# AER-RC/RRTMG_LW

Measured on AMD Instinct MI355X. Metric: columns/sec, 72-layer profiles, higher is better.
Workload: dtype f64 (transmittance / tfn codes and their LDS table f32); 1 GPU; 1000000 synthetic 72-layer columns, config 'cloudy' (icld=2: rtrnmr max-random overlap, idrv=0), sharded 1x1000000; ncol_total=1000000, nlay=72, columns_per_gpu=1000000, parallelism=columns/1, gather=none, kdata=stand-in (real k-data absent from the reference mount), sweeps=production

## Files before the change

rrtmg_lw_amd/csrc/kernels.hip:

```cpp
#include <hip/hip_runtime.h>
#include "kissjump.hpp"

#ifdef RRLW_TUNE
#define RRLW_BF_TUNE 1u
#else
#define RRLW_BF_TUNE 0u
#endif
#ifdef RRLW_G256
#define RRLW_BF_G256 8u
#else
#define RRLW_BF_G256 0u
#endif
#if defined(RRLW_LAYER_BLOCK) || defined(RRLW_STAGE_DOUBLES) || defined(RRLW_LAYER_WAVES) || defined(RRLW_LOAD_CHUNK) || defined(RRLW_MINOR_WIN) || \
    defined(RRLW_COLSORT_WIN) || defined(RRLW_SWEEPC_P0) || defined(RRLW_SWEEPC_P2D) || defined(RRLW_SWEEPC_WAVES_CAP) || defined(RRLW_SWEEPC_CODES) || \
    defined(RRLW_SWEEPZ_WAVES_G1) || defined(RRLW_SWEEPZ_WAVES_IDRV) || defined(RRLW_LAYER_STAMPS) || \
    defined(RRLW_DBG_DUMP)
#define RRLW_BF_GEOMETRY 16u
#else
#define RRLW_BF_GEOMETRY 0u
#endif

#include <algorithm>
#include <type_traits>
#include <utility>
// ... 566 lines not shown
};
struct Region {
    Key key; int a, b, rat;
    bool self_, for_;
    int planck_slot;
    bool frac_from_a;
    int nm; Minor m[3];
    int ncfc; int cfc_wx[2];
    Corr corr;
    int mult;
};
constexpr Minor NOM = {A_COL, 0, false, 0, 0, 0, 0, 0};
constexpr Region ZERO_REGION = {K_ZERO, 0, 0, 0, false, false, -1, false, 0, {NOM, NOM, NOM}, 0, {0, 0}, C_NONE, 0};

template <int B> struct BT;
#ifdef RRLW_G256
#define BAND_NG(NG_) 16
#else
#define BAND_NG(NG_) NG_
#endif
#define BAND_TRAITS(B_, NG_, LO, UP) \
    template <> struct BT<B_> { static constexpr int ng = BAND_NG(NG_); static constexpr Region lo = LO; static constexpr Region up = UP; };

#define R1(...) Region{__VA_ARGS__}
BAND_TRAITS(1, 10,
    R1(K_SINGLE, H2O, 0, 0, true, true, -1, false, 1, {{A_BRD_N2, BRD, false, 0, 0, 0, 0, 0}, NOM, NOM}, 0, {0, 0}, C_B1LO, 0),
    R1(K_SINGLE, H2O, 0, 0, false, true, -1, false, 1, {{A_BRD_N2, BRD, false, 0, 0, 0, 0, 0}, NOM, NOM}, 0, {0, 0}, C_B1UP, 0))
BAND_TRAITS(2, 12,
    R1(K_SINGLE, H2O, 0, 0, true, true, -1, false, 0, {NOM, NOM, NOM}, 0, {0, 0}, C_B2LO, 0),
    R1(K_SINGLE, H2O, 0, 0, false, true, -1, false, 0, {NOM, NOM, NOM}, 0, {0, 0}, C_NONE, 0))
BAND_TRAITS(3, 16,
    R1(K_BINARY, H2O, CO2, R_H2OCO2, true, true, 0, false, 1, {{A_ADJ, N2O, true, 2, 1.5, 0.5, 0.65, 0}, NOM, NOM}, 0, {0, 0}, C_NONE, 0),
    R1(K_BINARY, H2O, CO2, R_H2OCO2, false, true, 1, false, 1, {{A_ADJ, N2O, true, 3, 1.5, 0.5, 0.65, 0}, NOM, NOM}, 0, {0, 0}, C_NONE, 0))
BAND_TRAITS(4, 14,
    R1(K_BINARY, H2O, CO2, R_H2OCO2, true, true, 0, false, 0, {NOM, NOM, NOM}, 0, {0, 0}, C_NONE, 0),
    R1(K_BINARY, O3, CO2, R_O3CO2, false, false, 1, false, 0, {NOM, NOM, NOM}, 0, {0, 0}, C_NONE, 4))
BAND_TRAITS(5, 16,
    R1(K_BINARY, H2O, CO2, R_H2OCO2, true, true, 0, false, 1, {{A_COL, O3, true, 2, 0, 0, 0, 0}, NOM, NOM}, 1, {1, 0}, C_NONE, 0),
    R1(K_BINARY, O3, CO2, R_O3CO2, false, false, 1, false, 0, {NOM, NOM, NOM}, 1, {1, 0}, C_NONE, 0))
BAND_TRAITS(6, 8,
    R1(K_SINGLE, H2O, 0, 0, true, true, -1, false, 1, {{A_ADJ, CO2, false, 0, 3.0, 2.0, 0.77, 0}, NOM, NOM}, 2, {2, 3}, C_NONE, 0),
    R1(K_NONE, 0, 0, 0, false, false, -1, true, 0, {NOM, NOM, NOM}, 2, {2, 3}, C_NONE, 0))
BAND_TRAITS(7, 12,
    R1(K_BINARY, H2O, O3, R_H2OO3, true, true, 0, false, 1, {{A_ADJ, CO2, true, 2, 3.0, 3.0, 0.79, 0}, NOM, NOM}, 0, {0, 0}, C_NONE, 0),
    R1(K_SINGLE, O3, 0, 0, false, false, -1, false, 1, {{A_ADJ, CO2, false, 0, 3.0, 2.0, 0.79, 0}, NOM, NOM}, 0, {0, 0}, C_NONE, 7))
BAND_TRAITS(8, 8,
    R1(K_SINGLE, H2O, 0, 0, true, true, -1, false, 3,
       {{A_ADJ, CO2, false, 0, 3.0, 2.0, 0.65, 0}, {A_COL, O3, false, 0, 0, 0, 0, 0}, {A_COL, N2O, false, 0, 0, 0, 0, 0}}, 2, {3, 4}, C_NONE, 0),
    R1(K_SINGLE, O3, 0, 0, false, false, -1, false, 2,
       {{A_ADJ, CO2, false, 0, 3.0, 2.0, 0.65, 0}, {A_COL, N2O, false, 0, 0, 0, 0, 0}, NOM}, 2, {3, 4}, C_NONE, 0))
BAND_TRAITS(9, 12,
    R1(K_BINARY, H2O, CH4, R_H2OCH4, true, true, 0, false, 1, {{A_ADJ, N2O, true, 2, 1.5, 0.5, 0.65, 0}, NOM, NOM}, 0, {0, 0}, C_NONE, 0),
    R1(K_SINGLE, CH4, 0, 0, false, false, -1, false, 1, {{A_ADJ, N2O, false, 0, 1.5, 0.5, 0.65, 0}, NOM, NOM}, 0, {0, 0}, C_NONE, 0))
BAND_TRAITS(10, 6,
    R1(K_SINGLE, H2O, 0, 0, true, true, -1, false, 0, {NOM, NOM, NOM}, 0, {0, 0}, C_NONE, 0),
    R1(K_SINGLE, H2O, 0, 0, false, true, -1, false, 0, {NOM, NOM, NOM}, 0, {0, 0}, C_NONE, 0))
BAND_TRAITS(11, 8,
    R1(K_SINGLE, H2O, 0, 0, true, true, -1, false, 1, {{A_O2, O2, false, 0, 0, 0, 0, 0}, NOM, NOM}, 0, {0, 0}, C_NONE, 0),
    R1(K_SINGLE, H2O, 0, 0, false, true, -1, false, 1, {{A_O2, O2, false, 0, 0, 0, 0, 0}, NOM, NOM}, 0, {0, 0}, C_NONE, 0))
BAND_TRAITS(12, 8,
    R1(K_BINARY, H2O, CO2, R_H2OCO2, true, true, 0, false, 0, {NOM, NOM, NOM}, 0, {0, 0}, C_NONE, 0),
    ZERO_REGION)
BAND_TRAITS(13, 4,
    R1(K_BINARY, H2O, N2O, R_H2ON2O, true, true, 0, false, 2,
       {{A_ADJ, CO2, true, 2, 3.0, 2.0, 0.68, 3.55e-4}, {A_COL, CO, true, 4, 0, 0, 0, 0}, NOM}, 0, {0, 0}, C_NONE, 0),
    R1(K_NONE, 0, 0, 0, false, false, -1, false, 1, {{A_COL, O3, false, 0, 0, 0, 0, 0}, NOM, NOM}, 0, {0, 0}, C_NONE, 0))
BAND_TRAITS(14, 2,
    R1(K_SINGLE, CO2, 0, 0, true, true, -1, false, 0, {NOM, NOM, NOM}, 0, {0, 0}, C_NONE, 0),
    R1(K_SINGLE, CO2, 0, 0, false, false, -1, false, 0, {NOM, NOM, NOM}, 0, {0, 0}, C_NONE, 0))
BAND_TRAITS(15, 2,
    R1(K_BINARY, N2O, CO2, R_N2OCO2, true, true, 0, false, 1, {{A_BRD, BRD, true, 2, 0, 0, 0, 0}, NOM, NOM}, 0, {0, 0}, C_NONE, 0),
    ZERO_REGION)
BAND_TRAITS(16, 2,
    R1(K_BINARY, H2O, CH4, R_H2OCH4, true, true, 0, false, 0, {NOM, NOM, NOM}, 0, {0, 0}, C_NONE, 0),
    R1(K_SINGLE, CH4, 0, 0, false, false, -1, false, 0, {NOM, NOM, NOM}, 0, {0, 0}, C_NONE, 0))
#undef R1

__device__ const double kMult4[16] = {1, 1, 1, 1, 1, 1, 1, 0.92, 0.88, 1.07, 1.1, 0.99, 0.88, 0.943, 1, 1};
__device__ const double kMult7[16] = {1, 1, 1, 1, 1, 0.92, 0.88, 1.07, 1.1, 0.99, 0.855, 1, 1, 1, 1, 1};

struct LayerCoef {
    double f[NFIELD];
    int jp, jt, jt1, indself, indfor, indminor;
};

struct Spec { double speccomb, specparm, fs; int js; };
__device__ __forceinline__ Spec spec_calc(double cola, double rat, double colb, double mult, double oneminus)
{
    Spec s;
    s.speccomb = cola + rat * colb;
    s.specparm = fdiv(cola, s.speccomb);
    if (s.specparm >= oneminus) s.specparm = oneminus;
    const double specmult = mult * s.specparm;
    s.js = 1 + (int)specmult;
    s.fs = specmult - (double)(int)specmult;
    return s;
}

__device__ __forceinline__ void stencil6(double specparm, double fs, double fa, double fb, int &off, double (&w)[6])
{
    if (specparm < 0.125) {
        const double p = fs - 1, p2 = p * p, p4 = p2 * p2;
        const double fk0 = p4, fk1 = 1 - p - 2.0 * p4, fk2 = p + p4;
        off = 0;
        w[0] = fk0 * fa; w[1] = fk1 * fa; w[2] = fk2 * fa; w[3] = fk0 * fb; w[4] = fk1 * fb; w[5] = fk2 * fb;
    } else if (specparm > 0.875) {
        const double p = -fs, p2 = p * p, p4 = p2 * p2;
        const double fk0 = p4, fk1 = 1 - p - 2.0 * p4, fk2 = p + p4;
        off = -1;
        w[0] = fk2 * fa; w[1] = fk1 * fa; w[2] = fk0 * fa; w[3] = fk2 * fb; w[4] = fk1 * fb; w[5] = fk0 * fb;
    } else {
        off = 0;
        w[0] = (1. - fs) * fa; w[1] = fs * fa; w[2] = 0.0; w[3] = (1. - fs) * fb; w[4] = fs * fb; w[5] = 0.0;
    }
}

__host__ __device__ constexpr int region_nrows(const Region &R, bool lower)
{
    int n = 0;
    if (R.key == K_SINGLE) n += 4;
    else if (R.key == K_BINARY) n += lower ? 12 : 8;
    if (R.self_) n += 2;
    if (R.for_) n += 2;
    for (int i = 0; i < R.nm; i++) n += R.m[i].two_d ? 4 : 2;
    n += R.ncfc;
    return n;
}

__host__ __device__ constexpr int region_major_rows(const Region &R, bool lower)
{
    return R.key == K_SINGLE ? 4 : (R.key == K_BINARY ? (lower ? 12 : 8) : 0);
}
__host__ __device__ constexpr int region_minor_base(const Region &R, bool lower, int im)
{
    int n = region_major_rows(R, lower) + (R.self_ ? 2 : 0) + (R.for_ ? 2 : 0);
    for (int i = 0; i < im; i++) n += R.m[i].two_d ? 4 : 2;
    return n;
}

#ifdef RRLW_G256
__host__ __device__ constexpr int band_ng(int B) { return B >= 1 ? 16 : 16; }
#else
__host__ __device__ constexpr int band_ng(int B) { return B == 1 ? 10 : B == 2 ? 12 : B == 3 ? 16 : B == 4 ? 14 : B == 5 ? 16 : B == 6 ? 8 : B == 7 ? 12 :
                                                    B == 8 ? 8 : B == 9 ? 12 : B == 10 ? 6 : B == 11 ? 8 : B == 12 ? 8 : B == 13 ? 4 : 2; }
#endif
__host__ __device__ constexpr int band_nquad(int B) { return (band_ng(B) + 3) / 4; }
__host__ __device__ constexpr int band_qstart(int B)
{
    int s = 0;
    for (int b = 1; b < B; b++) s += band_nquad(b);
    return s;
}
constexpr int NQUAD = band_qstart(17);
__host__ __device__ constexpr int band_g0(int B)
{
    int s = 0;
    for (int b = 1; b < B; b++) s += band_ng(b);
    return s;
}
static_assert(band_g0(17) == NGPT, "g-point table");
static_assert(NQUAD == (NGPT == 140 ? 38 : 64), "quad table");

constexpr int NRATCHI = 6 * 59 + 7 * 59;
__shared__ double s_ratchi[NRATCHI];

template <int N>
struct Rows {
    unsigned off[N > 0 ? N : 1];
    double w[N > 0 ? N : 1];
    unsigned fw;
};

template <int B> constexpr unsigned lo_binary_mask() { return (BT<B>::lo.key == K_BINARY ? 1u << (B - 1) : 0u) | lo_binary_mask<B - 1>(); }
template <> constexpr unsigned lo_binary_mask<0>() { return 0u; }
template <int B> constexpr unsigned up_binary_mask() { return (BT<B>::up.key == K_BINARY ? 1u << (B - 1) : 0u) | up_binary_mask<B - 1>(); }
template <> constexpr unsigned up_binary_mask<0>() { return 0u; }
template <int B> constexpr unsigned up_zero_mask() { return (BT<B>::up.key == K_ZERO ? 1u << (B - 1) : 0u) | up_zero_mask<B - 1>(); }
template <> constexpr unsigned up_zero_mask<0>() { return 0u; }
template <int B> constexpr unsigned up_from_a_mask() { return (BT<B>::up.frac_from_a ? 1u << (B - 1) : 0u) | up_from_a_mask<B - 1>(); }
template <> constexpr unsigned up_from_a_mask<0>() { return 0u; }
constexpr unsigned LO_BINARY = lo_binary_mask<16>(), UP_BINARY = up_binary_mask<16>(), UP_ZERO = up_zero_mask<16>(), UP_FROM_A = up_from_a_mask<16>();
static_assert((UP_BINARY & ~LO_BINARY) == 0u, "fw slots are assigned by the lower region");
__host__ __device__ constexpr int popcnt_c(unsigned v) { int n = 0; for (; v; v &= v - 1) n++; return n; }
constexpr int NFW = popcnt_c(LO_BINARY);
__host__ __device__ constexpr int fw_slot(int B) { return popcnt_c(LO_BINARY & ((1u << (B - 1)) - 1u)); }

template <int B, bool LOWER, int N, int IM>
__device__ __forceinline__ void rows_prep_minor(const DevTables &T, const LayerCoef &C, Rows<N> &rw)
{
    constexpr Region R = LOWER ? BT<B>::lo : BT<B>::up;
    constexpr unsigned ng = BT<B>::ng;
    constexpr Minor M = R.m[IM];
    constexpr int I0 = region_minor_base(R, LOWER, IM);
    const BandLayout &L = T.band[B - 1];
    const double mf = C.f[F_MINORFRAC];
    double amount;
    if constexpr (M.amt == A_COL) amount = C.f[F_COLH2O + M.sp];
    else if constexpr (M.amt == A_BRD_N2) amount = C.f[F_COLBRD] * C.f[F_SCALEMINORN2];
    else if constexpr (M.amt == A_O2) amount = C.f[F_COLO2] * C.f[F_SCALEMINOR];
    else if constexpr (M.amt == A_BRD) amount = C.f[F_COLBRD] * C.f[F_SCALEMINOR];
    else {
        const double colx = C.f[F_COLH2O + M.sp], coldry = C.f[F_COLDRY];
        const double chiref = M.chiconst > 0. ? M.chiconst : s_ratchi[(T.sl.chi - T.sl.rat) + M.sp * 59 + C.jp];
        const double chi = fdiv(colx, coldry);
        const double ratx = fdiv(1.e20 * chi, chiref);
        amount = colx;
        if (ratx > M.thr) amount = (M.base + pow(ratx - M.base, M.expo)) * chiref * coldry * 1.e-20;
    }
    const unsigned slot = (unsigned)(LOWER ? L.minor_lo[IM] : L.minor_up[IM]);
    if constexpr (M.two_d) {
        constexpr unsigned nj = LOWER ? 9 : 5;
        const Spec sm = spec_calc(C.f[F_COLH2O + R.a], T.refrat[B - 1][M.refslot], C.f[F_COLH2O + R.b], LOWER ? 8. : 4., T.oneminus);
        const unsigned r = slot + ((unsigned)(C.indminor - 1) * nj + (unsigned)(sm.js - 1)) * ng;
        rw.off[I0] = r;                    rw.w[I0] = amount * ((1. - mf) * (1. - sm.fs));
        rw.off[I0 + 1] = r + ng;           rw.w[I0 + 1] = amount * ((1. - mf) * sm.fs);
        rw.off[I0 + 2] = r + nj * ng;      rw.w[I0 + 2] = amount * (mf * (1. - sm.fs));
        rw.off[I0 + 3] = r + nj * ng + ng; rw.w[I0 + 3] = amount * (mf * sm.fs);
    } else {
        const unsigned r = slot + (unsigned)(C.indminor - 1) * ng;
        rw.off[I0] = r;          rw.w[I0] = amount * (1. - mf);
        rw.off[I0 + 1] = r + ng; rw.w[I0 + 1] = amount * mf;
    }
}

template <int B, bool LOWER, int N>
__device__ __forceinline__ void rows_prep(const DevTables &T, const LayerCoef &C, Rows<N> &rw)
{
    constexpr Region R = LOWER ? BT<B>::lo : BT<B>::up;
    constexpr unsigned ng = BT<B>::ng;
    const BandLayout &L = T.band[B - 1];
    const int jp = C.jp, jt = C.jt, jt1 = C.jt1;
    const double *rat_tab = s_ratchi;
    rw.fw = 0u;
    if constexpr (R.key == K_ZERO) return;

    double corradj = 1.;
    if constexpr (R.corr == C_B1LO) { if (C.f[F_PAVEL] < 250.) corradj = 1. - 0.15 * (250. - C.f[F_PAVEL]) / 154.4; }
    else if constexpr (R.corr == C_B1UP) corradj = 1. - 0.15 * (C.f[F_PAVEL] / 95.6);
    else if constexpr (R.corr == C_B2LO) corradj = 1. - .05 * (C.f[F_PAVEL] - 100.) / 900.;

    if constexpr (R.key == K_SINGLE) {
        const unsigned r0 = LOWER ? ((jp - 1) * 5 + (jt - 1)) : ((jp - 13) * 5 + (jt - 1));
        const unsigned r1 = LOWER ? (jp * 5 + (jt1 - 1)) : ((jp - 12) * 5 + (jt1 - 1));
        const unsigned tab = (unsigned)(LOWER ? L.absa : L.absb);
        const double colk = C.f[F_COLH2O + R.a];
        rw.off[0] = tab + r0 * ng;       rw.w[0] = colk * C.f[F_FAC00];
        rw.off[1] = tab + (r0 + 1) * ng; rw.w[1] = colk * C.f[F_FAC10];
        rw.off[2] = tab + r1 * ng;       rw.w[2] = colk * C.f[F_FAC01];
        rw.off[3] = tab + (r1 + 1) * ng; rw.w[3] = colk * C.f[F_FAC11];
    } else if constexpr (R.key == K_BINARY) {
        const double cola = C.f[F_COLH2O + R.a], colb = C.f[F_COLH2O + R.b];
        const double rat = rat_tab[R.rat * 59 + (jp - 1)], rat_1 = rat_tab[R.rat * 59 + jp];
        constexpr double mult = LOWER ? 8. : 4.;
        const Spec s = spec_calc(cola, rat, colb, mult, T.oneminus);
        const Spec s1 = spec_calc(cola, rat_1, colb, mult, T.oneminus);
        if constexpr (LOWER) {
            const unsigned tab = (unsigned)L.absa;
            const int ind0 = ((jp - 1) * 5 + (jt - 1)) * 9 + s.js - 1;
            const int ind1 = (jp * 5 + (jt1 - 1)) * 9 + s1.js - 1;
            int so;
            double w6[6];
            stencil6(s.specparm, s.fs, C.f[F_FAC00], C.f[F_FAC10], so, w6);
            unsigned r = tab + (unsigned)(ind0 + so) * ng;
            rw.off[0] = r;           rw.w[0] = s.speccomb * w6[0];
            rw.off[1] = r + ng;      rw.w[1] = s.speccomb * w6[1];
            rw.off[2] = r + 2 * ng;  rw.w[2] = s.speccomb * w6[2];
            rw.off[3] = r + 9 * ng;  rw.w[3] = s.speccomb * w6[3];
            rw.off[4] = r + 10 * ng; rw.w[4] = s.speccomb * w6[4];
            rw.off[5] = r + 11 * ng; rw.w[5] = s.speccomb * w6[5];
            stencil6(s1.specparm, s1.fs, C.f[F_FAC01], C.f[F_FAC11], so, w6);
            r = tab + (unsigned)(ind1 + so) * ng;
            rw.off[6] = r;            rw.w[6] = s1.speccomb * w6[0];
            rw.off[7] = r + ng;       rw.w[7] = s1.speccomb * w6[1];
            rw.off[8] = r + 2 * ng;   rw.w[8] = s1.speccomb * w6[2];
            rw.off[9] = r + 9 * ng;   rw.w[9] = s1.speccomb * w6[3];
            rw.off[10] = r + 10 * ng; rw.w[10] = s1.speccomb * w6[4];
            rw.off[11] = r + 11 * ng; rw.w[11] = s1.speccomb * w6[5];
        } else {
            const unsigned tab = (unsigned)L.absb;
            const unsigned ind0 = ((jp - 13) * 5 + (jt - 1)) * 5 + s.js - 1;
            const unsigned ind1 = ((jp - 12) * 5 + (jt1 - 1)) * 5 + s1.js - 1;
            unsigned r = tab + ind0 * ng;
            rw.off[0] = r;          rw.w[0] = s.speccomb * ((1. - s.fs) * C.f[F_FAC00]);
            rw.off[1] = r + ng;     rw.w[1] = s.speccomb * (s.fs * C.f[F_FAC00]);
            rw.off[2] = r + 5 * ng; rw.w[2] = s.speccomb * ((1. - s.fs) * C.f[F_FAC10]);
            rw.off[3] = r + 6 * ng; rw.w[3] = s.speccomb * (s.fs * C.f[F_FAC10]);
            r = tab + ind1 * ng;
            rw.off[4] = r;          rw.w[4] = s1.speccomb * ((1. - s1.fs) * C.f[F_FAC01]);
            rw.off[5] = r + ng;     rw.w[5] = s1.speccomb * (s1.fs * C.f[F_FAC01]);
            rw.off[6] = r + 5 * ng; rw.w[6] = s1.speccomb * ((1. - s1.fs) * C.f[F_FAC11]);
            rw.off[7] = r + 6 * ng; rw.w[7] = s1.speccomb * (s1.fs * C.f[F_FAC11]);
        }
        const Spec sp = spec_calc(cola, T.refrat[B - 1][R.planck_slot], colb, mult, T.oneminus);
        unsigned q = (unsigned)(sp.fs * 268435456.0 + 0.5);
        if (q > 268435455u) q = 268435455u;
        rw.fw = ((unsigned)sp.js << 28) | q;
    }
    constexpr int IS = region_major_rows(R, LOWER);
    if constexpr (R.self_) {
        const unsigned r = (unsigned)L.selfref + (unsigned)(C.indself - 1) * ng;
        rw.off[IS] = r;          rw.w[IS] = C.f[F_SELFFAC] * (1. - C.f[F_SELFFRAC]);
        rw.off[IS + 1] = r + ng; rw.w[IS + 1] = C.f[F_SELFFAC] * C.f[F_SELFFRAC];
    }
    constexpr int IF = IS + (R.self_ ? 2 : 0);
    if constexpr (R.for_) {
        const unsigned r = (unsigned)L.forref + (unsigned)(C.indfor - 1) * ng;
// ... 1600 lines not shown
__device__ __forceinline__ void sweep_stage_lut(const DevTables &T, unsigned char *smem, int tid, int nth)
{
    const double2 *src = reinterpret_cast<const double2 *>(T.stat + T.sl.lutf);
    double2 *dst = reinterpret_cast<double2 *>(smem);
    constexpr int NLUT = SWEEP_LUT_BYTES / 16;
    for (int i0 = tid; i0 < NLUT; i0 += 8 * nth) {
        double2 v[8];
#pragma unroll
        for (int k = 0; k < 8; k++) v[k] = src[min(i0 + k * nth, NLUT - 1)];
#pragma unroll
        for (int k = 0; k < 8; k++) if (i0 + k * nth < NLUT) dst[i0 + k * nth] = v[k];
    }
}
__device__ __forceinline__ void sweep_stage_band(const DevTables &T, double (*s_pl)[184], double (*s_fr)[16], int B, bool alt16, bool lo_bin, bool up_bin,
                                                 int tid, int nth)
{
    const double *tp = alt16 ? T.stat + T.sl.totplk16 : T.stat + T.sl.totplnk + 181 * (B - 1);
    const double *tq = T.stat + T.sl.totplnk + 181 * 15;
    for (int i = tid; i < 181; i += nth) { s_pl[0][i] = tp[i]; s_pl[1][i] = tq[i]; }
    const int ng = T.band[B - 1].ng, fa = T.band[B - 1].fracrefa, fb = T.band[B - 1].fracrefb;
    const int na = lo_bin ? 9 : 1, nb = up_bin ? 5 : 1;
    for (int i = tid; i < 16 * 16; i += nth) {
        const int r = i >> 4, g = i & 15;
        double v = 0.0;
        if (g < ng) {
            if (r < 9) { if (r < na) v = T.ktab[fa + r * ng + g]; }
            else if (r < 14 && fb >= 0 && r - 9 < nb) v = T.ktab[fb + (r - 9) * ng + g];
        }
        s_fr[r][g] = v;
    }
}
#ifndef RRLW_SWEEPC_P0
#define RRLW_SWEEPC_P0 6, 4, 3, 2
#endif
#ifndef RRLW_SWEEPC_P2D
#define RRLW_SWEEPC_P2D 3, 2, 1, 1
#endif
#ifndef RRLW_SWEEPC_WAVES_CAP
#define RRLW_SWEEPC_WAVES_CAP 4
#endif
__host__ __device__ constexpr int sweepc_waves(int NQ, int PHASE, bool IDRV)
{
    const int row = PHASE == 1 ? 0 : (PHASE == 0 && !IDRV) ? 1 : (PHASE == 2 && IDRV) ? 3 : 2;
    const int tab[4][4] = {{7, 5, 4, 3}, {RRLW_SWEEPC_P0}, {5, 3, 2, 1}, {RRLW_SWEEPC_P2D}};
    const int w = tab[row][NQ - 1];
    return w < RRLW_SWEEPC_WAVES_CAP ? w : RRLW_SWEEPC_WAVES_CAP;
}
constexpr int NGROUP_MAX = 8;
constexpr int SWEEPC_BAND_BYTES = SWEEP_PL_BYTES + SWEEP_FR_BYTES;
__host__ __device__ constexpr int sweepc_nval(int PHASE, bool IDRV) { return (PHASE == 2 ? 2 : 1) * ((IDRV && PHASE != 1) ? 2 : 1); }
#ifndef RRLW_SWEEPC_CODES
#define RRLW_SWEEPC_CODES 2
#endif
constexpr int SWEEPC_LDS_MAX = 160 * 1024;
__host__ __device__ constexpr int sweepc_lds_bytes(int PHASE, bool IDRV, int nb, int nsb, int NT = 1)
{
    return SWEEP_LUT_BYTES + nb * SWEEPC_BAND_BYTES + 2 * sweepc_nval(PHASE, IDRV) * nb * NT * RRLW_SWEEPC_CODES * nsb * 64 * 8;
}
__host__ __device__ constexpr int sweepc_nt(int NQ, int PHASE)
{
    return (NQ == 4 && (PHASE == 2 || PHASE == 0)) ? 2 : 1;
}
__host__ __device__ constexpr int sweepc_group_cap(int NQ)
{
    int cap = 5;
    for (int ph = 0; ph < 3; ph++)
        for (int i = 0; i < 2; i++) {
            if (ph == 1 && i == 1) continue;
            const bool idrv = i == 1;
            const int nt = sweepc_nt(NQ, ph), w = 4 * sweepc_waves(NQ / nt, ph, idrv) / nt;
            if (w < cap) cap = w;
            while (cap > 1 && sweepc_lds_bytes(ph, idrv, cap, 1, nt) > SWEEPC_LDS_MAX) cap--;
        }
    return cap;
}
__host__ __device__ constexpr int sweepc_nsb(int NQ, int PHASE, bool IDRV, int nb)
{
    const int nt = sweepc_nt(NQ, PHASE);
    int nsb = nsb_fit(4 * sweepc_waves(NQ / nt, PHASE, IDRV) / (nb * nt));
    while (nsb > 1 && sweepc_lds_bytes(PHASE, IDRV, nb, nsb, nt) > SWEEPC_LDS_MAX) nsb = nsb_fit(nsb - 1);
    return nsb;
}

template <int G> struct SweepcLev { double tl, tz; unsigned w; };

__device__ __forceinline__ double one_minus(double x)
{
    double t = 1.0 - x;
    asm("" : "+v"(t));
    return t;
}
__device__ __forceinline__ double times(double x, double y)
{
    double t = x * y;
    asm("" : "+v"(t));
    return t;
}

template <int NQ, int PHASE, bool IDRV, int NT = 1, bool SPEC = false>
__global__ __launch_bounds__(256 * sweepc_waves(NQ / NT, PHASE, IDRV), sweepc_waves(NQ / NT, PHASE, IDRV)) void k_sweepc(DevTables T, Workspace W, SweepArgs a)
{
    static_assert(NQ % NT == 0 && (NT == 1 || NT == 2), "threads per band");
    constexpr int G = NQ / NT, NG = 4 * G, NC = RRLW_SWEEPC_CODES;
    constexpr bool DOWN = PHASE != 2, UP = PHASE != 1, TWO = PHASE == 2;
    constexpr int NVAL = sweepc_nval(PHASE, IDRV);
    extern __shared__ __align__(16) unsigned char smem[];
    const int hgrp = (PHASE == 0 && !a.cfree) ? 0 : __builtin_amdgcn_readfirstlane(W.hgrp[(blockIdx.x * blockDim.z) / SORT_GROUP]);
    if (a.cfree && (PHASE == 0) != (hgrp == 0)) return;
    const int tx = threadIdx.x, ty = __builtin_amdgcn_readfirstlane(threadIdx.y), sub = __builtin_amdgcn_readfirstlane(threadIdx.z);
    const int bi = ty / NT, part = ty % NT;
    const int ny = blockDim.y, nb = ny / NT, nsb = blockDim.z, ncw = 64 * nsb;
    const float2 *s_lut = reinterpret_cast<const float2 *>(smem);
    double (*s_pl)[184] = reinterpret_cast<double (*)[184]>(smem + SWEEP_LUT_BYTES + bi * SWEEPC_BAND_BYTES);
    double (*s_fr)[16] = reinterpret_cast<double (*)[16]>(smem + SWEEP_LUT_BYTES + bi * SWEEPC_BAND_BYTES + SWEEP_PL_BYTES);
    double *red = reinterpret_cast<double *>(smem + SWEEP_LUT_BYTES + nb * SWEEPC_BAND_BYTES);
    const int slot = blockIdx.x * nsb + sub;
    const int cblock = (PHASE == 0 && !a.cfree) ? slot : __builtin_amdgcn_readfirstlane(W.order[slot]);
    const int col = cblock * 64 + tx;
    const int bsel = a.split ? (int)blockIdx.y : 0;
    const unsigned long long bands = a.bands >> (4 * bsel);
    const int B = (int)((bands >> (4 * bi)) & 15ull) + 1;
    const bool incol = col < a.ncol;
    const int colc = incol ? col : a.ncol - 1;
    const int quad = __builtin_amdgcn_readfirstlane(band_qstart(B) + part * G);
    const int g0 = NG * part;
    const int pc = pcol(W, colc);
    const size_t gc = (size_t)a.col0 + pc;
    const int nlay = W.nlay, nct = a.nct;
    const size_t ncb = W.ncolb;
    const bool alt16 = (B == 16 && a.istart == 16);
    const bool lo_bin = (LO_BINARY >> (B - 1)) & 1u, up_bin = (UP_BINARY >> (B - 1)) & 1u;
    const bool any_bin = lo_bin || up_bin;
    const int base_up = ((UP_ZERO >> (B - 1)) & 1u) ? 14 : (((UP_FROM_A >> (B - 1)) & 1u) ? 0 : 9);
    sweep_stage_lut(T, smem, (sub * ny + ty) * 64 + tx, 64 * ny * nsb);
    sweep_stage_band(T, s_pl, s_fr, B, alt16, lo_bin, up_bin, (sub * NT + part) * 64 + tx, NT * ncw);
    __syncthreads();
    const int lo = PHASE == 0 ? 1 : hgrp + 1;
    const size_t qstride = (size_t)nlay * ncb;
    const unsigned *__restrict__ sC = W.scr[S_CODE] + (size_t)quad * qstride * CODE_WORDS;
    const unsigned *__restrict__ sFw = W.fw + (size_t)fw_slot(B) * nlay * ncb;
    const bool moved = pmoved(W, colc);
    const double *__restrict__ tlay = moved ? W.tlayc : a.tlay + a.col0;
    const double *__restrict__ tlev = moved ? W.tlevc : a.tlev + a.col0;
    const size_t tstride = moved ? ncb : (size_t)nct;
    const unsigned offc = (unsigned)colc * (unsigned)CODE_BYTES, off8p = (unsigned)colc * 8u, off4 = (unsigned)colc * 4u;
    const size_t pcb = (size_t)W.pcb;
    const size_t gslab = (size_t)(a.group + bsel) * (nlay + 1) * pcb;
    double *__restrict__ gdn1 = W.gdn1 + gslab;
    double *__restrict__ gup1 = W.gup1 + gslab;
    Part2 *__restrict__ gup = W.gup + gslab;
    Part2 *__restrict__ gdp = W.gdp + gslab;
    const unsigned so8 = (unsigned)col * 8u, so16 = (unsigned)col * 16u;
    const int laytrop = W.laytrop[colc];
    const double *tp0 = s_pl[0], *tp1 = s_pl[1];
    double2 *hand = reinterpret_cast<double2 *>(W.hand) + ((size_t)quad * ncb + colc) * 2;
    const size_t hstream = (size_t)NQUAD * ncb * 2;

    constexpr bool SOFF = PHASE != 1;
    const unsigned ncb32 = (unsigned)ncb, tstr32 = (unsigned)tstride;
    auto fill_t = [&](auto bin_tag, int lev, int zoff, SweepcLev<G> &q) {
        const int l = min(max(lev, 1), nlay);
        if constexpr (SOFF) {
            const unsigned r = (unsigned)(l - 1);
            q.tl = bload_f64(row_ptr(tlay, r, tstr32), off8p);
            q.tz = bload_f64(row_ptr(tlev, r + (unsigned)zoff, tstr32), off8p);
            if constexpr (decltype(bin_tag)::value) q.w = bload_u32(sFw, off4, r * ncb32 * 4u);
        } else {
            q.tl = bload_f64(tlay + tstride * (l - 1), off8p);
            q.tz = bload_f64(tlev + tstride * (l - 1 + zoff), off8p);
            if constexpr (decltype(bin_tag)::value) q.w = bload_u32(sFw + (size_t)(l - 1) * ncb, off4);
        }
    };
    auto ld_c = [&](int lev, int k) -> pk4 {
        const int l = min(max(lev, 1), nlay);
        if constexpr (SOFF) return bload_pk4_nt(sC + (size_t)k * qstride * CODE_WORDS, offc, (unsigned)(l - 1) * ncb32 * (unsigned)CODE_BYTES);
        else return bload_pk4_nt(sC + ((size_t)k * qstride + (size_t)(l - 1) * ncb) * CODE_WORDS, offc);
    };
    auto frac_row = [&](int lev, unsigned fwv, double &fpl) -> const double * {
        const bool lower = lev <= laytrop;
        if (any_bin) {
            const unsigned w = (lower ? lo_bin : up_bin) ? fwv : 0x10000000u;
            const int r0 = clampi((lower ? 0 : base_up) + (int)(w >> 28) - 1, 0, 14);
            fpl = (double)(w & 0x0fffffffu) * (1.0 / 268435456.0);
            return &s_fr[r0][g0];
        }
        fpl = 0.0;
        return &s_fr[lower ? 0 : base_up][g0];
    };

    const unsigned rlane = (unsigned)(sub * 64 + tx);
    const unsigned vstride = (unsigned)(ny * NC * ncw), rband = (unsigned)(ty * NC * ncw);
    unsigned bufoff = 0u;
    auto red_put = [&](int c, int val, double v) { red[bufoff + val * vstride + rband + (unsigned)(c * ncw) + rlane] = v; };
    auto round_end = [&](auto dn_tag, int lev0, int nvalid) {
#pragma clang fp contract(off)
        constexpr bool DN = decltype(dn_tag)::value;
        constexpr int NV = DN ? 1 : NVAL;
        __syncthreads();
        for (int c = ty; c < nvalid; c += ny) {
            const int lvl = DN ? lev0 - c - 1 : lev0 + c;
            double sv[NV];
#pragma unroll
            for (int val = 0; val < NV; val++) {
                const double *r = red + (bufoff + val * vstride + (unsigned)(c * ncw) + rlane);
                const bool deriv = IDRV && !DN && val >= (TWO ? 2 : 1);
                double sum = 0.0;
                for (int q = 0; q < nb; q++) {
                    double pq = r[(unsigned)(q * NT * NC * ncw)];
                    if constexpr (NT == 2) pq = pq + r[(unsigned)((q * NT + 1) * NC * ncw)];
                    const int bq = (int)((bands >> (4 * q)) & 15ull);
                    double v = (pq * 0.5) * T.delwave[bq];
                    if (deriv) v = v * T.fluxfac;
                    sum = q == 0 ? v : sum + v;
                    if constexpr (SPEC) {
                        if (incol && !deriv) {
                            const size_t o = spec_at(gc, lvl, bq + 1, nlay, nct);
                            const double f = v * T.fluxfac;
                            if (DN) { a.dflxs[o] = f; if (a.dflxcs) a.dflxcs[o] = f; }
                            else if (val == 0) { a.uflxs[o] = f; if (!TWO && a.uflxcs) a.uflxcs[o] = f; }
                            else if (a.uflxcs) a.uflxcs[o] = f;
                        }
                    }
                }
                sv[val] = sum;
            }
            if (incol) {
                if constexpr (DN) bstore_f64(gdn1 + (size_t)lvl * pcb, so8, sv[0]);
                else {
                    if constexpr (TWO) bstore_f64x2(gup + (size_t)lvl * pcb, so16, sv[0], sv[1]);
                    else bstore_f64(gup1 + (size_t)lvl * pcb, so8, sv[0]);
                    if constexpr (IDRV) bstore_f64x2(gdp + (size_t)lvl * pcb, so16, TWO ? sv[2] : sv[1], TWO ? sv[3] : sv[1]);
                }
            }
        }
        bufoff = bufoff ? 0u : NVAL * vstride;
    };

    double rad[NG], radc[TWO ? NG : 1], drad[IDRV ? NG : 1], dradc[(IDRV && TWO) ? NG : 1];
#pragma unroll
    for (int j = 0; j < NG; j++) rad[j] = 0.0;

    SweepcLev<G> cur;
    cur.w = 0u;
    pk4 cc[G][NC];
    auto level = [&](auto bin_tag, auto dn_tag, int lev, int slot) {
        constexpr bool BIN = decltype(bin_tag)::value, DN = decltype(dn_tag)::value;
        constexpr int dir = DN ? -1 : 1;
        double fpl;
        const double *row = frac_row(lev, cur.w, fpl);
        const double blay = planck_at(tp0, tp0, cur.tl);
        const double dpl = planck_at(tp0, (DN && alt16 && lev == 1) ? tp1 : tp0, cur.tz) - blay;
        fill_t(bin_tag, lev + dir, DN ? 0 : 1, cur);
        double qs[G], qsc[G], qd[G], qdc[G];
#pragma unroll
        for (int k = 0; k < G; k++) {
            pk4 pk;
#pragma unroll
            for (int c = 0; c < NC; c++) if (c == slot) pk = cc[k][c];
            const scr4 ck = unpack4(pk);
            unsigned orw = pk.w[0];
#pragma unroll
            for (int i = 1; i < CODE_WORDS; i++) orw |= pk.w[i];
            const bool thin = wave_all_thin(orw);
            float fa[4], ft[4];
            if (thin) {
#pragma unroll
                for (int jj = 0; jj < 4; jj++) decode_thin(ck.v[jj], fa[jj], ft[jj]);
            } else {
                float2 e[4];
#pragma unroll
                for (int jj = 0; jj < 4; jj++) e[jj] = s_lut[code_index(ck.v[jj])];
#pragma unroll
                for (int jj = 0; jj < 4; jj++) decode_f32(ck.v[jj], e[jj], fa[jj], ft[jj]);
            }
            const pk4 nx = ld_c(lev + NC * dir, k);
#pragma unroll
            for (int c = 0; c < NC; c++) if (c == slot) cc[k][c] = nx;
#pragma unroll
            for (int jj = 0; jj < 4; jj++) {
                const int j = 4 * k + jj;
                const double atr = (double)fa[jj], tfn = (double)ft[jj];
                double fr = row[j];
                if constexpr (BIN) fr = fma(fpl, row[16 + j] - fr, fr);
                const double bb = fr * fma(tfn, dpl, blay);
                rad[j] = fma(bb - rad[j], atr, rad[j]);
                if constexpr (TWO && !DN) radc[j] = fma(bb - radc[j], atr, radc[j]);
                if constexpr (IDRV && !DN) {
                    const double tr = one_minus(atr);
                    drad[j] = times(drad[j], tr);
                    if constexpr (TWO) dradc[j] = times(dradc[j], tr);
                }
            }
            qs[k] = (rad[4 * k] + rad[4 * k + 1]) + (rad[4 * k + 2] + rad[4 * k + 3]);
            if constexpr (TWO && !DN) qsc[k] = (radc[4 * k] + radc[4 * k + 1]) + (radc[4 * k + 2] + radc[4 * k + 3]);
            if constexpr (IDRV && !DN) {
                qd[k] = (drad[4 * k] + drad[4 * k + 1]) + (drad[4 * k + 2] + drad[4 * k + 3]);
                if constexpr (TWO) qdc[k] = (dradc[4 * k] + dradc[4 * k + 1]) + (dradc[4 * k + 2] + dradc[4 * k + 3]);
            }
#pragma unroll
            for (int jj = 0; jj < 4; jj++) {
                asm volatile("" : "+v"(rad[4 * k + jj]));
                if constexpr (TWO && !DN) asm volatile("" : "+v"(radc[4 * k + jj]));
                if constexpr (IDRV && !DN) asm volatile("" : "+v"(drad[4 * k + jj]));
                if constexpr (IDRV && TWO && !DN) asm volatile("" : "+v"(dradc[4 * k + jj]));
            }
        }
        auto tree = [&](const double (&q)[G]) -> double {
            if constexpr (G == 1) return q[0];
            else if constexpr (G == 2) return q[0] + q[1];
            else if constexpr (G == 3) return (q[0] + q[1]) + q[2];
            else return (q[0] + q[1]) + (q[2] + q[3]);
        };
        red_put(slot, 0, tree(qs));
        if constexpr (TWO && !DN) red_put(slot, 1, tree(qsc));
        if constexpr (IDRV && !DN) {
            red_put(slot, TWO ? 2 : 1, tree(qd));
            if constexpr (TWO) red_put(slot, 3, tree(qdc));
        }
    };
    auto sweep = [&](auto bin_tag, auto dn_tag) {
        constexpr bool DN = decltype(dn_tag)::value;
        constexpr int dir = DN ? -1 : 1;
        const int first = DN ? nlay : lo, count = nlay - lo + 1;
#pragma unroll
        for (int c = 0; c < NC; c++) {
            if (c == NC - 1) fill_t(bin_tag, first, DN ? 0 : 1, cur);
#pragma unroll
            for (int k = 0; k < G; k++) cc[k][c] = ld_c(first + c * dir, k);
        }
        int n = 0;
        for (; n + NC <= count; n += NC) {
#pragma unroll
            for (int c = 0; c < NC; c++) level(bin_tag, dn_tag, first + (n + c) * dir, c);
            round_end(dn_tag, first + n * dir, NC);
        }
        const int rem = count - n;
#pragma unroll
        for (int c = 0; c < NC - 1; c++) {
            if (c < rem) level(bin_tag, dn_tag, first + (n + c) * dir, c);
        }
        if (rem > 0) round_end(dn_tag, first + n * dir, rem);
    };
    using std::true_type;
    using std::false_type;

    if constexpr (DOWN) {
        if (incol && ty == 0) bstore_f64(gdn1 + (size_t)nlay * pcb, so8, 0.0);
        if constexpr (SPEC) {
            if (incol && part == 0) {
                const size_t o = spec_at(gc, nlay, B, nlay, nct);
                a.dflxs[o] = 0.0;
                if (a.dflxcs) a.dflxcs[o] = 0.0;
            }
        }
        if (any_bin) sweep(true_type{}, true_type{}); else sweep(false_type{}, true_type{});
    }
    if constexpr (PHASE == 1) {
        if (incol) {
#pragma unroll
            for (int k = 0; k < G; k++) {
                hand[(size_t)k * ncb * 2] = make_double2(rad[4 * k], rad[4 * k + 1]);
                hand[(size_t)k * ncb * 2 + 1] = make_double2(rad[4 * k + 2], rad[4 * k + 3]);
            }
        }
        return;
    }

    if constexpr (PHASE == 0) {
        const double reflect = 1. - a.emis[gc + (size_t)nct * (B - 1)];
        const double pb = W.percol[(size_t)(PC_PLANKBND + B - 1) * ncb + colc];
        const double dpb = IDRV ? W.percol[(size_t)(PC_DPLANKBND + B - 1) * ncb + colc] : 0.0;
        double fpl;
        const double *row = frac_row(1, any_bin ? bload_u32(sFw, off4) : 0u, fpl);
        double usum = 0.0, dusum = 0.0;
#pragma unroll
        for (int j = 0; j < NG; j++) {
            const double fr = any_bin ? fma(fpl, row[16 + j] - row[j], row[j]) : row[j];
            rad[j] = fma(reflect, rad[j], fr * pb);
            usum = usum + rad[j];
            if constexpr (IDRV) { drad[j] = times(fr, dpb); dusum = dusum + drad[j]; }
        }
        if (a.cfree) {
            double qs[G], qd[G];
#pragma unroll
            for (int k = 0; k < G; k++) {
                qs[k] = 0.0; qd[k] = 0.0;
#pragma unroll
                for (int jj = 0; jj < 4; jj++) {
                    qs[k] = qs[k] + rad[4 * k + jj];
                    if constexpr (IDRV) qd[k] = qd[k] + drad[4 * k + jj];
                }
            }
            if constexpr (G == 1) { usum = qs[0]; dusum = qd[0]; }
            else if constexpr (G == 2) { usum = qs[0] + qs[1]; dusum = qd[0] + qd[1]; }
            else if constexpr (G == 3) { usum = (qs[0] + qs[1]) + qs[2]; dusum = (qd[0] + qd[1]) + qd[2]; }
            else { usum = (qs[0] + qs[1]) + (qs[2] + qs[3]); dusum = (qd[0] + qd[1]) + (qd[2] + qd[3]); }
        }
        red_put(0, 0, usum);
        if constexpr (IDRV) red_put(0, 1, dusum);
        round_end(false_type{}, 0, 1);
    } else {
#pragma unroll
        for (int k = 0; k < G; k++) {
            const double2 *h = hand + (size_t)k * ncb * 2;
            const double2 a0 = h[hstream], a1 = h[hstream + 1], c0 = h[2 * hstream], c1 = h[2 * hstream + 1];
            rad[4 * k] = a0.x; rad[4 * k + 1] = a0.y; rad[4 * k + 2] = a1.x; rad[4 * k + 3] = a1.y;
            if constexpr (TWO) { radc[4 * k] = c0.x; radc[4 * k + 1] = c0.y; radc[4 * k + 2] = c1.x; radc[4 * k + 3] = c1.y; }
            if constexpr (IDRV) {
                const double2 d0 = h[3 * hstream], d1 = h[3 * hstream + 1], e0 = h[4 * hstream], e1 = h[4 * hstream + 1];
                drad[4 * k] = d0.x; drad[4 * k + 1] = d0.y; drad[4 * k + 2] = d1.x; drad[4 * k + 3] = d1.y;
                if constexpr (TWO) { dradc[4 * k] = e0.x; dradc[4 * k + 1] = e0.y; dradc[4 * k + 2] = e1.x; dradc[4 * k + 3] = e1.y; }
            }
        }
    }
    if constexpr (UP) {
        if (any_bin) sweep(true_type{}, false_type{}); else sweep(false_type{}, false_type{});
    }
}

__host__ __device__ constexpr int sweepz_nt(int NQ) { return NQ; }
#ifndef RRLW_SWEEPZ_WAVES_G1
#define RRLW_SWEEPZ_WAVES_G1 3
#endif
#ifndef RRLW_SWEEPZ_WAVES_IDRV
#define RRLW_SWEEPZ_WAVES_IDRV 2
#endif
__host__ __device__ constexpr int sweepz_waves(int , bool IDRV = false)
{
    return IDRV ? RRLW_SWEEPZ_WAVES_IDRV : RRLW_SWEEPZ_WAVES_G1;
}
__host__ __device__ constexpr int sweepz_lds_bytes(int nb, int nsb, int NT, bool IDRV = false)
{
    return SWEEP_LUT_BYTES + nb * SWEEPC_BAND_BYTES + 2 * (IDRV ? 4 : 2) * nb * NT * RRLW_SWEEPC_CODES * nsb * 64 * 8;
}
__host__ __device__ constexpr int sweepz_nsb(int NQ, int nb, bool IDRV = false)
{
    const int nt = sweepz_nt(NQ);
    int nsb = nsb_fit(4 * sweepz_waves(NQ, IDRV) / (nb * nt));
    while (nsb > 1 && sweepz_lds_bytes(nb, nsb, nt, IDRV) > SWEEPC_LDS_MAX) nsb = nsb_fit(nsb - 1);
    return nsb;
}

__host__ __device__ constexpr int sweepz_group_cap(int NQ, bool IDRV)
{
    const int nt = sweepz_nt(NQ);
    int cap = 4 * sweepz_waves(NQ, IDRV) / nt;
    if (cap < 1) cap = 1;
    while (cap > 1 && sweepz_lds_bytes(cap, 1, nt, IDRV) > SWEEPC_LDS_MAX) cap--;
    return cap;
}

struct SweepzLev { double tl, tz, cf; unsigned w, flag; };

template <int NQ, int MODE, bool IDRV = false, bool SPEC = false>
__global__ __launch_bounds__(256 * sweepz_waves(NQ, IDRV), sweepz_waves(NQ, IDRV)) void k_sweepz(DevTables T, Workspace W, SweepArgs a)
{
    static_assert(MODE >= 1 && MODE <= 4, "modes of the cloud-zone sweep");
    constexpr int G = 1, NT = sweepz_nt(NQ), NG = 4 * G, NC = RRLW_SWEEPC_CODES, NVAL = IDRV ? 4 : 2;
    constexpr int NS2 = MODE == 2 ? NG : 1;
    constexpr int NSD = IDRV ? NG : 1;
    extern __shared__ __align__(16) unsigned char smem[];
    const int ltop = __builtin_amdgcn_readfirstlane(W.hgrp[(blockIdx.x * blockDim.z) / SORT_GROUP]);
    if (a.cfree && ltop == 0) return;
    const int tx = threadIdx.x, ty = __builtin_amdgcn_readfirstlane(threadIdx.y), sub = __builtin_amdgcn_readfirstlane(threadIdx.z);
    const int bi = ty / NT, part = ty % NT;
    const int ny = blockDim.y, nb = ny / NT, nsb = blockDim.z, ncw = 64 * nsb;
    const float2 *s_lut = reinterpret_cast<const float2 *>(smem);
    double (*s_pl)[184] = reinterpret_cast<double (*)[184]>(smem + SWEEP_LUT_BYTES + bi * SWEEPC_BAND_BYTES);
    double (*s_fr)[16] = reinterpret_cast<double (*)[16]>(smem + SWEEP_LUT_BYTES + bi * SWEEPC_BAND_BYTES + SWEEP_PL_BYTES);
    double *red = reinterpret_cast<double *>(smem + SWEEP_LUT_BYTES + nb * SWEEPC_BAND_BYTES);
    const int cblock = __builtin_amdgcn_readfirstlane(W.order[blockIdx.x * nsb + sub]);
    const int col = cblock * 64 + tx;
    const int bsel = a.split ? (int)blockIdx.y : 0;
    const unsigned long long bands = a.bands >> (4 * bsel);
    const int B = (int)((bands >> (4 * bi)) & 15ull) + 1;
    const bool incol = col < a.ncol;
    const int colc = incol ? col : a.ncol - 1;
    const int quad = __builtin_amdgcn_readfirstlane(band_qstart(B) + part * G);
    const int g0 = NG * part;
    const int pc = pcol(W, colc);
    const size_t gc = (size_t)a.col0 + pc;
    const int nlay = W.nlay, nct = a.nct;
    const size_t ncb = W.ncolb;
    const bool alt16 = (B == 16 && a.istart == 16);
    const bool lo_bin = (LO_BINARY >> (B - 1)) & 1u, up_bin = (UP_BINARY >> (B - 1)) & 1u;
    const bool any_bin = lo_bin || up_bin;
    const int base_up = ((UP_ZERO >> (B - 1)) & 1u) ? 14 : (((UP_FROM_A >> (B - 1)) & 1u) ? 0 : 9);
    sweep_stage_lut(T, smem, (sub * ny + ty) * 64 + tx, 64 * ny * nsb);
    sweep_stage_band(T, s_pl, s_fr, B, alt16, lo_bin, up_bin, (sub * NT + part) * 64 + tx, NT * ncw);
    __syncthreads();
    const size_t qstride = (size_t)nlay * ncb;
    const unsigned *__restrict__ sC = W.scr[S_CODE] + (size_t)quad * qstride * CODE_WORDS;
    const unsigned *__restrict__ sCt = W.scr[S_CODET] + (size_t)quad * qstride * CODE_WORDS;
    const unsigned *__restrict__ sFw = W.fw + (size_t)fw_slot(B) * nlay * ncb;
    const int *__restrict__ sFlag = W.cflag;
    const bool moved = pmoved(W, colc);
    const double *__restrict__ tlay = moved ? W.tlayc : a.tlay + a.col0;
    const double *__restrict__ tlev = moved ? W.tlevc : a.tlev + a.col0;
    const double *__restrict__ cldf = moved ? W.cldfc : a.cldfrac + a.col0;
    const size_t tstride = moved ? ncb : (size_t)nct;
    const unsigned off16 = (unsigned)colc * 16u, offc = (unsigned)colc * (unsigned)CODE_BYTES, off8 = (unsigned)colc * 8u, off4 = (unsigned)colc * 4u;
    const size_t pcb = (size_t)W.pcb;
    const size_t gslab = (size_t)(a.group + bsel) * (nlay + 1) * pcb;
    Part2 *__restrict__ gdn = W.gdn + gslab;
    Part2 *__restrict__ gup = W.gup + gslab;
    Part2 *__restrict__ gdp = W.gdp + gslab;
    const unsigned so16 = (unsigned)col * 16u;
    const int laytrop = W.laytrop[colc];
    const double *tp0 = s_pl[0], *tp1 = s_pl[1];
    double2 *hand = reinterpret_cast<double2 *>(W.hand) + ((size_t)quad * ncb + colc) * 2;
    const size_t hstream = (size_t)NQUAD * ncb * 2;
    const bool colcloud = (bload_u32(sFlag, off4) & 8u) != 0;
    const int ig0 = band_g0(B) + g0, mw0 = ig0 >> 5, mw1 = mw0 < 4 ? mw0 + 1 : 4;
    const int nvalid = max(0, min(NG, band_ng(B) - g0));

    auto clampl = [&](int lev) { return min(max(lev, 1), nlay); };
    const unsigned ncb32 = (unsigned)ncb, tstr32 = (unsigned)tstride;
    auto fill_t = [&](auto bin_tag, auto lite_tag, int lev, int zoff, SweepzLev &q) {
        const unsigned r = (unsigned)(clampl(lev) - 1);
        q.tl = bload_f64(row_ptr(tlay, r, tstr32), off8);
        q.tz = bload_f64(row_ptr(tlev, r + (unsigned)zoff, tstr32), off8);
        if constexpr (!decltype(lite_tag)::value) {
            q.cf = bload_f64(row_ptr(cldf, r, tstr32), off8);
            q.flag = bload_u32(sFlag, off4, (r + 1u) * ncb32 * 4u);
        }
        if constexpr (decltype(bin_tag)::value) q.w = bload_u32(sFw, off4, r * ncb32 * 4u);
    };
    auto ld_c = [&](const unsigned *base, int lev, int k) -> pk4 {
        return bload_pk4_nt(base + (size_t)k * qstride * CODE_WORDS, offc, (unsigned)(clampl(lev) - 1) * ncb32 * (unsigned)CODE_BYTES);
    };
    auto frac_row = [&](int lev, unsigned fwv, double &fpl) -> const double * {
        const bool lower = lev <= laytrop;
        if (any_bin) {
            const unsigned w = (lower ? lo_bin : up_bin) ? fwv : 0x10000000u;
            const int r0 = clampi((lower ? 0 : base_up) + (int)(w >> 28) - 1, 0, 14);
            fpl = (double)(w & 0x0fffffffu) * (1.0 / 268435456.0);
            return &s_fr[r0][g0];
        }
        fpl = 0.0;
        return &s_fr[lower ? 0 : base_up][g0];
    };

    const unsigned rlane = (unsigned)(sub * 64 + tx);
    const unsigned vstride = (unsigned)(ny * NC * ncw), rband = (unsigned)(ty * NC * ncw);
    unsigned bufoff = 0u;
    auto red_put = [&](int c, int val, double v) { red[bufoff + val * vstride + rband + (unsigned)(c * ncw) + rlane] = v; };
    auto round_end = [&](auto dn_tag, int lev0, int nvalid) __attribute__((always_inline)) {
#pragma clang fp contract(off)
        constexpr bool DN = decltype(dn_tag)::value;
        __syncthreads();
        constexpr int NV = DN ? 2 : NVAL;
        for (int c = ty; c < nvalid; c += ny) {
            const int lvl = DN ? lev0 - c - 1 : lev0 + c;
            double sv[NV];
#pragma unroll
            for (int val = 0; val < NV; val++) {
                const double *r = red + (bufoff + val * vstride + (unsigned)(c * ncw) + rlane);
                double sum = 0.0;
                for (int q = 0; q < nb; q++) {
                    double pq = r[(unsigned)(q * NT * NC * ncw)];
                    if constexpr (NT >= 2) pq = pq + r[(unsigned)((q * NT + 1) * NC * ncw)];
                    if constexpr (NT == 3) pq = pq + r[(unsigned)((q * NT + 2) * NC * ncw)];
                    if constexpr (NT == 4) pq = pq + (r[(unsigned)((q * NT + 2) * NC * ncw)] + r[(unsigned)((q * NT + 3) * NC * ncw)]);
                    const int bq = (int)((bands >> (4 * q)) & 15ull);
                    double v = (pq * 0.5) * T.delwave[bq];
                    if (val >= 2) v = v * T.fluxfac;
                    sum = q == 0 ? v : sum + v;
                    if constexpr (SPEC) {
                        if (incol && val < 2) {
// ... 924 lines not shown
```

Baseline: 17.85 million columns/s.

## Split sweeps at block-max tropopause to skip fraction interpolation aloft

Each block computes a wave- and block-wide maximum of laytrop across its sub-columns. The up and down radiative sweeps are then split into a below-tropopause segment that does binary fraction interpolation and an aloft segment that uses a fixed upper-atmosphere fraction row with no per-level weight loads. Template tags pick the segment variants at compile time according to each band-group's binary-interpolation mask. The aim is to cut per-level global loads and branches above the tropopause. In exchange it adds a small reduction prologue, more code instantiations and register pressure, and forced inlining.

```diff
diff --git a/rrtmg_lw_amd/csrc/kernels.hip b/rrtmg_lw_amd/csrc/kernels.hip
--- a/rrtmg_lw_amd/csrc/kernels.hip
+++ b/rrtmg_lw_amd/csrc/kernels.hip
@@ -742,6 +742,12 @@
     return s;
 }
 constexpr int NQUAD = band_qstart(17);
+__host__ __device__ constexpr unsigned nquad_mask(int nq)
+{
+    unsigned m = 0u;
+    for (int b = 1; b <= 16; b++) if (band_nquad(b) == nq) m |= 1u << (b - 1);
+    return m;
+}
 __host__ __device__ constexpr int band_g0(int B)
 {
     int s = 0;
@@ -2648,13 +2654,28 @@
     Part2 *__restrict__ gdp = W.gdp + gslab;
     const unsigned so8 = (unsigned)col * 8u, so16 = (unsigned)col * 16u;
     const int laytrop = W.laytrop[colc];
+    constexpr unsigned MINE = nquad_mask(NQ);
+    constexpr bool SPLIT = PHASE != 1 && (MINE & ~UP_BINARY) != 0u;
+    constexpr bool HAS_UP_BIN = (MINE & UP_BINARY) != 0u, HAS_LO_BIN = (MINE & LO_BINARY & ~UP_BINARY) != 0u, HAS_NO_BIN = (MINE & ~LO_BINARY) != 0u;
+    int ltrop = nlay;
+    if constexpr (SPLIT) {
+        ltrop = laytrop;
+        for (int s = 0; s < nsb; s++) {
+            if (s == sub) continue;
+            const int sl = blockIdx.x * nsb + s;
+            const int cb = (PHASE == 0 && !a.cfree) ? sl : __builtin_amdgcn_readfirstlane(W.order[sl]);
+            ltrop = max(ltrop, W.laytrop[min(cb * 64 + tx, a.ncol - 1)]);
+        }
+        for (int o = 32; o >= 1; o >>= 1) ltrop = max(ltrop, __shfl_xor(ltrop, o, 64));
+        ltrop = __builtin_amdgcn_readfirstlane(ltrop);
+    }
     const double *tp0 = s_pl[0], *tp1 = s_pl[1];
     double2 *hand = reinterpret_cast<double2 *>(W.hand) + ((size_t)quad * ncb + colc) * 2;
     const size_t hstream = (size_t)NQUAD * ncb * 2;
 
     constexpr bool SOFF = PHASE != 1;
     const unsigned ncb32 = (unsigned)ncb, tstr32 = (unsigned)tstride;
-    auto fill_t = [&](auto bin_tag, int lev, int zoff, SweepcLev<G> &q) {
+    auto fill_t = [&](auto bin_tag, int lev, int zoff, SweepcLev<G> &q) __attribute__((always_inline)) {
         const int l = min(max(lev, 1), nlay);
         if constexpr (SOFF) {
             const unsigned r = (unsigned)(l - 1);
@@ -2667,12 +2688,21 @@
             if constexpr (decltype(bin_tag)::value) q.w = bload_u32(sFw + (size_t)(l - 1) * ncb, off4);
         }
     };
-    auto ld_c = [&](int lev, int k) -> pk4 {
+    auto fill_w = [&](int lev) __attribute__((always_inline)) -> unsigned {
+        const int l = min(max(lev, 1), nlay);
+        if constexpr (SOFF) return bload_u32(sFw, off4, (unsigned)(l - 1) * ncb32 * 4u);
+        else return bload_u32(sFw + (size_t)(l - 1) * ncb, off4);
+    };
+    auto ld_c = [&](int lev, int k) __attribute__((always_inline)) -> pk4 {
         const int l = min(max(lev, 1), nlay);
         if constexpr (SOFF) return bload_pk4_nt(sC + (size_t)k * qstride * CODE_WORDS, offc, (unsigned)(l - 1) * ncb32 * (unsigned)CODE_BYTES);
         else return bload_pk4_nt(sC + ((size_t)k * qstride + (size_t)(l - 1) * ncb) * CODE_WORDS, offc);
     };
-    auto frac_row = [&](int lev, unsigned fwv, double &fpl) -> const double * {
+    auto frac_row = [&](auto aloft_tag, int lev, unsigned fwv, double &fpl) __attribute__((always_inline)) -> const double * {
+        if constexpr (decltype(aloft_tag)::value) {
+            fpl = 0.0;
+            return &s_fr[base_up][g0];
+        }
         const bool lower = lev <= laytrop;
         if (any_bin) {
             const unsigned w = (lower ? lo_bin : up_bin) ? fwv : 0x10000000u;
@@ -2687,8 +2717,8 @@
     const unsigned rlane = (unsigned)(sub * 64 + tx);
     const unsigned vstride = (unsigned)(ny * NC * ncw), rband = (unsigned)(ty * NC * ncw);
     unsigned bufoff = 0u;
-    auto red_put = [&](int c, int val, double v) { red[bufoff + val * vstride + rband + (unsigned)(c * ncw) + rlane] = v; };
-    auto round_end = [&](auto dn_tag, int lev0, int nvalid) {
+    auto red_put = [&](int c, int val, double v) __attribute__((always_inline)) { red[bufoff + val * vstride + rband + (unsigned)(c * ncw) + rlane] = v; };
+    auto round_end = [&](auto dn_tag, int lev0, int nvalid) __attribute__((always_inline)) {
 #pragma clang fp contract(off)
         constexpr bool DN = decltype(dn_tag)::value;
         constexpr int NV = DN ? 1 : NVAL;
@@ -2739,11 +2769,12 @@
     SweepcLev<G> cur;
     cur.w = 0u;
     pk4 cc[G][NC];
-    auto level = [&](auto bin_tag, auto dn_tag, int lev, int slot) {
+    auto level = [&](auto bin_tag, auto aloft_tag, auto dn_tag, int lev, int slot) __attribute__((always_inline)) {
         constexpr bool BIN = decltype(bin_tag)::value, DN = decltype(dn_tag)::value;
+        static_assert(!(BIN && decltype(aloft_tag)::value), "an aloft level does not interpolate");
         constexpr int dir = DN ? -1 : 1;
         double fpl;
-        const double *row = frac_row(lev, cur.w, fpl);
+        const double *row = frac_row(aloft_tag, lev, cur.w, fpl);
         const double blay = planck_at(tp0, tp0, cur.tl);
         const double dpl = planck_at(tp0, (DN && alt16 && lev == 1) ? tp1 : tp0, cur.tz) - blay;
         fill_t(bin_tag, lev + dir, DN ? 0 : 1, cur);
@@ -2801,7 +2832,7 @@
                 if constexpr (IDRV && TWO && !DN) asm volatile("" : "+v"(dradc[4 * k + jj]));
             }
         }
-        auto tree = [&](const double (&q)[G]) -> double {
+        auto tree = [&](const double (&q)[G]) __attribute__((always_inline)) -> double {
             if constexpr (G == 1) return q[0];
             else if constexpr (G == 2) return q[0] + q[1];
             else if constexpr (G == 3) return (q[0] + q[1]) + q[2];
@@ -2814,28 +2845,65 @@
             if constexpr (TWO) red_put(slot, 3, tree(qdc));
         }
     };
-    auto sweep = [&](auto bin_tag, auto dn_tag) {
+    auto prime = [&](auto bin_tag, auto dn_tag, int first) __attribute__((always_inline)) {
         constexpr bool DN = decltype(dn_tag)::value;
         constexpr int dir = DN ? -1 : 1;
-        const int first = DN ? nlay : lo, count = nlay - lo + 1;
 #pragma unroll
         for (int c = 0; c < NC; c++) {
             if (c == NC - 1) fill_t(bin_tag, first, DN ? 0 : 1, cur);
 #pragma unroll
             for (int k = 0; k < G; k++) cc[k][c] = ld_c(first + c * dir, k);
         }
+    };
+    auto segment = [&](auto bin_tag, auto aloft_tag, auto dn_tag, int first, int count) __attribute__((always_inline)) {
+        constexpr bool DN = decltype(dn_tag)::value;
+        constexpr int dir = DN ? -1 : 1;
         int n = 0;
         for (; n + NC <= count; n += NC) {
 #pragma unroll
-            for (int c = 0; c < NC; c++) level(bin_tag, dn_tag, first + (n + c) * dir, c);
+            for (int c = 0; c < NC; c++) level(bin_tag, aloft_tag, dn_tag, first + (n + c) * dir, c);
             round_end(dn_tag, first + n * dir, NC);
         }
         const int rem = count - n;
 #pragma unroll
         for (int c = 0; c < NC - 1; c++) {
-            if (c < rem) level(bin_tag, dn_tag, first + (n + c) * dir, c);
+            if (c < rem) level(bin_tag, aloft_tag, dn_tag, first + (n + c) * dir, c);
         }
         if (rem > 0) round_end(dn_tag, first + n * dir, rem);
+    };
+    const int count = nlay - lo + 1, ltb = min(max(ltrop, lo - 1), nlay);
+    const int n_aloft_dn = ((nlay - ltb) / NC) * NC;
+    const int n_below_up = min(((ltb - lo + 1 + NC - 1) / NC) * NC, count);
+    auto sweep = [&](auto dn_tag) __attribute__((always_inline)) {
+        constexpr bool DN = decltype(dn_tag)::value;
+        using std::true_type;
+        using std::false_type;
+        const int first = DN ? nlay : lo;
+        if constexpr (!SPLIT) {
+            if ((HAS_UP_BIN || HAS_LO_BIN) && (!HAS_NO_BIN || any_bin)) { prime(true_type{}, dn_tag, first); segment(true_type{}, false_type{}, dn_tag, first, count); }
+            else { prime(false_type{}, dn_tag, first); segment(false_type{}, false_type{}, dn_tag, first, count); }
+        } else if (HAS_UP_BIN && up_bin) {
+            prime(true_type{}, dn_tag, first);
+            segment(true_type{}, false_type{}, dn_tag, first, count);
+        } else if constexpr (DN) {
+            const bool interp = HAS_LO_BIN && (!HAS_NO_BIN || any_bin);
+            if (interp && n_aloft_dn == 0) prime(true_type{}, dn_tag, first);
+            else prime(false_type{}, dn_tag, first);
+            segment(false_type{}, true_type{}, dn_tag, first, n_aloft_dn);
+            if (interp) {
+                if (n_aloft_dn > 0) cur.w = fill_w(first - n_aloft_dn);
+                segment(true_type{}, false_type{}, dn_tag, first - n_aloft_dn, count - n_aloft_dn);
+            } else if constexpr (HAS_NO_BIN) segment(false_type{}, false_type{}, dn_tag, first - n_aloft_dn, count - n_aloft_dn);
+        } else {
+            if (HAS_LO_BIN && (!HAS_NO_BIN || any_bin)) {
+                prime(true_type{}, dn_tag, first);
+                segment(true_type{}, false_type{}, dn_tag, first, n_below_up);
+            } else if constexpr (HAS_NO_BIN) {
+                prime(false_type{}, dn_tag, first);
+                segment(false_type{}, false_type{}, dn_tag, first, n_below_up);
+            }
+            segment(false_type{}, true_type{}, dn_tag, first + n_below_up, count - n_below_up);
+        }
     };
     using std::true_type;
     using std::false_type;
@@ -2849,7 +2917,7 @@
                 if (a.dflxcs) a.dflxcs[o] = 0.0;
             }
         }
-        if (any_bin) sweep(true_type{}, true_type{}); else sweep(false_type{}, true_type{});
+        sweep(true_type{});
     }
     if constexpr (PHASE == 1) {
         if (incol) {
@@ -2867,7 +2935,7 @@
         const double pb = W.percol[(size_t)(PC_PLANKBND + B - 1) * ncb + colc];
         const double dpb = IDRV ? W.percol[(size_t)(PC_DPLANKBND + B - 1) * ncb + colc] : 0.0;
         double fpl;
-        const double *row = frac_row(1, any_bin ? bload_u32(sFw, off4) : 0u, fpl);
+        const double *row = frac_row(false_type{}, 1, any_bin ? bload_u32(sFw, off4) : 0u, fpl);
         double usum = 0.0, dusum = 0.0;
 #pragma unroll
         for (int j = 0; j < NG; j++) {
@@ -2910,7 +2978,7 @@
         }
     }
     if constexpr (UP) {
-        if (any_bin) sweep(true_type{}, false_type{}); else sweep(false_type{}, false_type{});
+        sweep(false_type{});
     }
 }
 
```

Result: no change. 17.94 million columns/s, median of 6 (+0.5%).
